# yehonatan145/PatternMatching

Hardware: AMD Instinct MI355X
Metric: GB/s stream scanned + matches/sec, snort.dict, 1/2/4/8 MI355X vs CPU ref (higher is better)
Workload: dtype u8

## Files before the change

patternmatching_amd/csrc/pm_kernels.hip:

```cpp
#include <type_traits>

#include <algorithm>

#include "pm_kernels.h"
#include "pm_streamgen.h"

namespace {

#ifdef RT_PLAIN_STORES
#define RT_OUT_STORE(v, p) (*(p) = (v))
#else
#define RT_OUT_STORE(v, p) __builtin_nontemporal_store((v), (p))
#endif
constexpr int RT_THREADS = 1024;
constexpr int RT_WAVES = RT_THREADS / 64;
constexpr int RT_T2_U16 = 65536;
constexpr int RT_FILTER_WORDS = 4096;
constexpr int RT_F3_WORDS = 256;
constexpr int RT_F2_WORDS = 2048;
constexpr uint32_t RT_QCAP = 64;
constexpr uint32_t RT_ROUND = 40;
constexpr int RT_CHUNK = 1024;
constexpr uint32_t CONT16 = 0x8000u;
constexpr uint32_t CONT32 = 0x80000000u;
// ... 105 lines not shown
        } else {
            const uint32_t ch = wide_child(t.wide[(size_t)R.z * 4 + (c >> 6)], c);
            if (ch == ~0u) return R.y;
            node = ch;
        }
        ++d;
    }
}

__device__ __forceinline__ uint32_t rt_slot1(uint32_t k, uint32_t bits) { return rt_hash(k) >> (32 - bits); }
__device__ __forceinline__ uint32_t rt_slot2(uint32_t k, uint32_t bits) { return (k * 0x85EBCA77u) >> (32 - bits); }

template <bool FOLD = false>
__device__ __forceinline__ uint32_t rt_from_d2(const uint8_t* __restrict__ text, const RtDev& t, uint32_t key24,
                                               uint32_t c3, uint32_t best2, int64_t i, int64_t avail) {
    const uint32_t want = T3H_VALID | key24;
    uint4 e = t.t3h[rt_slot1(key24, t.t3h_bits)];
    if ((e.x & 0x1FFFFFFu) != want) {
        e = t.t3h[rt_slot2(key24, t.t3h_bits)];
        if ((e.x & 0x1FFFFFFu) != want) return best2;
    }
    const uint32_t kind = e.x >> 25;
    if (kind == 0 || avail < 4) return e.y;
    if (kind == 1) {
        const uint32_t nch = e.z >> 24;
        const uint32_t k = c3 == (e.z & 0xFFu) ? 0u : c3 == ((e.z >> 8) & 0xFFu) ? 1u : c3 == ((e.z >> 16) & 0xFFu) ? 2u : 3u;
        if (k >= nch) return e.y;
        if (nch > 1) return rt_deep<FOLD>(text, t, e.w + k, i, avail, 4);
        if (!(e.w & CONT32)) return e.w;
        return rt_deep<FOLD>(text, t, e.w & 0x7FFFFFFFu, i, avail, 4);
    }
    return rt_deep<FOLD>(text, t, e.w & 0x7FFFFFFFu, i, avail, 3);
}

template <bool FOLD = false>
__device__ uint32_t rt_one(const uint8_t* __restrict__ text, const uint16_t* s_t, const RtDev& t, int64_t i,
                           int64_t stream_start) {
    const int64_t avail = i - stream_start + 1;
    const uint32_t c0 = rt_byte<FOLD>(text, i);
    if (avail == 1) return t.t12[65536 + c0];
    const uint32_t c1 = rt_byte<FOLD>(text, i - 1);
    const uint32_t v = s_t[(c0 << 8) | c1];
    if (!(v & CONT16) || avail == 2) return v & 0x7FFFu;
    return rt_from_d2<FOLD>(text, t, rt_byte<FOLD>(text, i - 2) | (c1 << 8) | (c0 << 16),
                            avail >= 4 ? rt_byte<FOLD>(text, i - 3) : 0u, v & 0x7FFFu, i, avail);
}

template <int OUTW>
__device__ __forceinline__ void put_id(void* out, int64_t k, uint32_t v) {
    if (OUTW == 4) reinterpret_cast<uint32_t*>(out)[k] = v;
    if (OUTW == 2) reinterpret_cast<uint16_t*>(out)[k] = (uint16_t)v;
}

template <int I, int N, class F>
__device__ __forceinline__ void unroll_for(F&& f) {
    if constexpr (I < N) {
        f(std::integral_constant<int, I>{});
        unroll_for<I + 1, N>(f);
    }
}

using tu32x2 = __attribute__((ext_vector_type(2))) unsigned int;
using tu32x4 = __attribute__((ext_vector_type(4))) unsigned int;

constexpr int RT_PROBE_G = 4;
constexpr int RT_TAIL_SLOTS = 4;
constexpr uint32_t RT_D4 = 1u << 30;
enum : uint32_t { TS_EMPTY = 0, TS_ENTRY, TS_REC, TS_WIDE };

struct TailSlot {
    uint32_t st;
    uint32_t pos;
    uint32_t av;
    uint32_t node, dd;
    uint32_t c;
    uint32_t tlo, thi;
    int32_t twa;
    const tu32x4* pa;
    const tu32x2* pb;
    tu32x4 A;
    tu32x2 B;
};

template <int OUTW, bool kProbeOnly = false, int SLOTS = RT_TAIL_SLOTS>
__device__ __forceinline__ uint32_t rt_tail(const uint8_t* __restrict__ text, int64_t stream_start, int64_t pos0,
                                        void* __restrict__ out, const RtDev& t, const uint32_t* s_f2,
                                        uint32_t* sp, uint32_t sn, int lane, uint32_t& cnt) {
    const uint8_t* const tb = text + pos0;
    const int64_t ctx64 = pos0 - stream_start;
    const uint32_t ctx = ctx64 > 1024 ? 1024u : (uint32_t)ctx64;
    const tu32x4* const dummy4 = reinterpret_cast<const tu32x4*>(t.filt);
    const tu32x2* const dummy2 = reinterpret_cast<const tu32x2*>(t.filt);
    const tu32x4* const T3 = reinterpret_cast<const tu32x4*>(t.t3h);
    const tu32x4* const RC = reinterpret_cast<const tu32x4*>(t.rec);
    const tu32x4* const WD = reinterpret_cast<const tu32x4*>(t.wide);
    tu32x2* const items = reinterpret_cast<tu32x2*>(sp);

    uint32_t nwalk = 0;
    for (uint32_t base = 0; base < sn; base += 64 * RT_PROBE_G) {
        tu32x2 it[RT_PROBE_G];
        tu32x4 e[RT_PROBE_G];
        bool act[RT_PROBE_G];
        unroll_for<0, RT_PROBE_G>([&](auto g) __attribute__((always_inline)) {
            const uint32_t idx = base + 64 * g + lane;
            it[g] = idx < sn ? items[idx] : tu32x2{0u, 0u};
            act[g] = idx < sn && rt_stage2_hit(rt_stage2_load(s_f2, it[g].x)) != 0u;
        });
        unroll_for<0, RT_PROBE_G>([&](auto g) __attribute__((always_inline)) {
            e[g] = act[g] ? T3[rt_slot1(it[g].x >> 8, t.t3h_bits)] : *dummy4;
        });
        bool need2[RT_PROBE_G];
        bool any2 = false;
        unroll_for<0, RT_PROBE_G>([&](auto g) __attribute__((always_inline)) {
            const uint32_t want = T3H_VALID | (it[g].x >> 8);
            need2[g] = act[g] && (e[g].x & 0x1FFFFFFu) != want && (e[g].x & T3H_VALID);
            any2 |= need2[g];
        });
        if (__ballot(any2)) {
            unroll_for<0, RT_PROBE_G>([&](auto g) __attribute__((always_inline)) {
                if (need2[g]) e[g] = T3[rt_slot2(it[g].x >> 8, t.t3h_bits)];
            });
        }
        unroll_for<0, RT_PROBE_G>([&](auto g) __attribute__((always_inline)) {
            const tu32x4 E = e[g];
            const uint32_t key = it[g].x, pw = it[g].y, off = pw & RT_POSMASK;
            const bool match = act[g] && (E.x & 0x1FFFFFFu) == (T3H_VALID | (key >> 8));
            const uint32_t kind = E.x >> 25, nch = E.z >> 24, c3 = key & 0xFFu;
            const uint32_t j = c3 == (E.z & 0xFFu) ? 0u : c3 == ((E.z >> 8) & 0xFFu) ? 1u
                             : c3 == ((E.z >> 16) & 0xFFu) ? 2u : 3u;
            const bool deep4 = off + ctx >= 3;
            const bool inl = kind == 1 && j < nch && nch == 1 && !(E.w & CONT32);
            const bool walk = match && deep4 && ((kind == 1 && j < nch && !inl) || kind == 2);
            const uint32_t node = (kind == 2 || nch == 1) ? E.w & 0x7FFFFFFFu : E.w + j;
            const uint32_t ans = (deep4 && inl) ? E.w : E.y;
            if (match && !walk) {
                cnt += (uint32_t)(ans != 0u) - (pw >> 31);
                if (OUTW) put_id<OUTW>(out, (int64_t)off, ans);
            }
            const uint64_t m = __ballot(walk);
            if (walk) items[nwalk + wave_prefix(m)] = tu32x2{node, (pw & ~RT_D4) | (kind == 1 ? RT_D4 : 0u)};
            nwalk += (uint32_t)__popcll(m);
        });
    }
    if (!nwalk || kProbeOnly) return nwalk;
    __builtin_amdgcn_s_waitcnt(0);
    __builtin_amdgcn_fence(__ATOMIC_ACQUIRE, "agent");

    TailSlot S[SLOTS];
    unroll_for<0, SLOTS>([&](auto I) __attribute__((always_inline)) {
        TailSlot& z = S[I];
        z.st = TS_EMPTY;
        z.pos = z.av = z.node = z.dd = z.c = z.tlo = z.thi = 0;
        z.twa = 0;
        z.pa = dummy4;
        z.pb = dummy2;
        z.A = tu32x4{0u, 0u, 0u, 0u};
        z.B = tu32x2{0u, 0u};
    });
    uint32_t nxt = 0;
    for (;;) {
        bool busy = false;
        unroll_for<0, SLOTS>([&](auto I) __attribute__((always_inline)) {
            TailSlot& z = S[I];
            const bool need = z.st == TS_EMPTY;
            const uint64_t m = __ballot(need);
            const uint32_t idx = nxt + wave_prefix(m);
            if (need && idx < nwalk) {
                z.st = TS_ENTRY;
                z.c = idx & 1u;
                z.pa = reinterpret_cast<const tu32x4*>(items + (idx & ~1u));
                z.pb = dummy2;
            }
            nxt += (uint32_t)__popcll(m);
            if (nxt > nwalk) nxt = nwalk;
            busy |= z.st != TS_EMPTY;
        });
        if (!__ballot(busy)) break;
        unroll_for<0, SLOTS>([&](auto I) __attribute__((always_inline)) {
            TailSlot& z = S[I];
            z.A = *z.pa;
            z.B = *z.pb;
        });
        unroll_for<0, SLOTS>([&](auto I) __attribute__((always_inline)) {
            TailSlot& z = S[I];
            const uint32_t st = z.st;
            const tu32x4 A = z.A;
            const uint32_t en = z.c ? A.z : A.x, ep = z.c ? A.w : A.y;
            const uint32_t off = z.pos & RT_POSMASK;
            const int32_t rq = (int32_t)off - (int32_t)z.dd;
            const bool reload = rq < z.twa || rq >= z.twa + 8;
            const uint32_t rlo = reload ? z.B.x : z.tlo, rhi = reload ? z.B.y : z.thi;
            const int32_t rta = reload ? (rq & ~7) : z.twa;
            const uint32_t ro = (uint32_t)(rq - rta);
            const uint32_t c = ((ro & 4 ? rhi : rlo) >> (8 * (ro & 3))) & 0xFFu;
            const uint32_t rkind = rec_kind(A), first = A.x & 0xFFFFFFu;
            const uint32_t jr = rec_kid_index(A, c);
            const bool rend = z.dd >= z.av;
            const bool rnext = !rend && rkind == RT_REC_KIDS_K && jr != ((A.x >> 24) & 63u);
            const bool rwide = !rend && rkind == RT_REC_WIDE_K;
            const uint64_t win = ((uint64_t)rhi << 32 | rlo) << (8 * (7 - ro));
            const uint64_t dif = win ^ ((uint64_t)A.w << 32 | A.z);
            const uint32_t meq = dif ? (uint32_t)__builtin_clzll(dif) >> 3 : 8u;
            const uint32_t clen = (A.x >> 24) & 63u;
            const uint32_t cav = z.av > z.dd ? z.av - z.dd : 0u;
            const uint32_t clim = min(min(clen, ro + 1u), cav);
            const uint32_t cm = min(meq, clim);
            const bool cnext = rkind == RT_REC_CHAIN_K && cm >= 1u && (cm == clen || (cm == ro + 1u && cm < cav));
            const uint32_t wnode = wide_child(A, z.c);
            const bool wnext = wnode != ~0u;

            uint32_t nst = TS_EMPTY;
            bool fin = false;
            uint32_t ans = A.w;
            if (st == TS_ENTRY) {
                nst = TS_REC;
                z.node = en;
                z.dd = (ep & RT_D4) ? 4u : 3u;
                z.pos = ep & ~RT_D4;
                const uint32_t o = ep & RT_POSMASK;
                z.av = o + ctx + 1 > 1024u ? 1024u : o + ctx + 1;
                z.twa = INT32_MIN / 2;
            }
            if (st == TS_REC) {
                nst = (rnext || cnext) ? TS_REC : rwide ? TS_WIDE : TS_EMPTY;
                fin = !rnext && !rwide && !cnext;
                ans = A.y;
                z.tlo = rlo;
                z.thi = rhi;
                z.twa = rta;
                z.node = cnext ? first + cm - 1u : first + jr;
                z.dd += rnext ? 1u : cnext ? cm : 0u;
                z.c = c;
            }
            if (st == TS_WIDE) {
                nst = wnext ? TS_REC : TS_EMPTY;
                fin = !wnext;
                z.node = wnode;
                z.dd += 1;
            }
            if (fin) {
                cnt += (uint32_t)(ans != 0u) - (z.pos >> 31);
                if (OUTW) put_id<OUTW>(out, (int64_t)(z.pos & RT_POSMASK), ans);
            }
            z.st = nst;
            const int32_t nq = (int32_t)(z.pos & RT_POSMASK) - (int32_t)z.dd;
            const bool nreload = z.dd < z.av && (nq < z.twa || nq >= z.twa + 8);
            const tu32x4* pa = dummy4;
            const tu32x2* pb = dummy2;
            if (nst == TS_REC) {
                pa = RC + z.node;
                if (nreload) pb = reinterpret_cast<const tu32x2*>(tb + (nq & ~7));
            }
            if (nst == TS_WIDE) pa = WD + (size_t)A.z * 4 + (c >> 6);
            z.pa = pa;
            z.pb = pb;
        });
    }
    return nwalk;
}

template <int V, int OUTW, bool EF = false>
__global__ __launch_bounds__(RT_THREADS) void rt_scan_kernel(const uint8_t* __restrict__ text, int64_t stream_start,
                                                             int64_t pos0, int64_t n, void* __restrict__ out,
                                                             unsigned long long* __restrict__ count, RtDev t) {
    static_assert(V == 0 || V == 2, "product kernel (0) or streaming floor (2)");
    constexpr bool kT8 = V == 0 && OUTW == 0;
    constexpr int kLdsWords = kT8 ? RT_T2_U16 / 4 + RT_F2_WORDS + 2 * RT_WAVES * RT_QCAP
                                  : RT_FILTER_WORDS + RT_T2_U16 / 2 + RT_F2_WORDS + 2 * RT_WAVES * RT_QCAP;
    __shared__ __attribute__((aligned(16))) uint32_t s_lds[kLdsWords];
    uint32_t* const s_f = s_lds;
    const uint8_t* const s_t8 = reinterpret_cast<const uint8_t*>(s_lds);
    const uint16_t* const s_t = kT8 ? t.t12 : reinterpret_cast<uint16_t*>(s_lds + RT_FILTER_WORDS);
    uint32_t* const s_f2 = s_lds + (kT8 ? RT_T2_U16 / 4 : RT_FILTER_WORDS + RT_T2_U16 / 2);
    uint32_t(*const s_qkey)[RT_QCAP] = reinterpret_cast<uint32_t(*)[RT_QCAP]>(s_f2 + RT_F2_WORDS);
    uint32_t(*const s_qpos)[RT_QCAP] = s_qkey + RT_WAVES;
    {
        const uint4* fsrc = reinterpret_cast<const uint4*>(t.filt);
        if (kT8) {
            const uint2* src = reinterpret_cast<const uint2*>(t.t12);
            for (int k = threadIdx.x; k < RT_T2_U16 / 4; k += RT_THREADS) {
                const uint2 v = src[k];
                const uint32_t e[4] = {v.x & 0xFFFFu, v.x >> 16, v.y & 0xFFFFu, v.y >> 16};
                uint32_t w = 0;
#pragma unroll
                for (int q = 0; q < 4; ++q) {
                    const uint32_t nz = (e[q] & 0x7FFFu) != 0u, cand = !nz && (e[q] & CONT16);
                    w |= (nz | cand << 1) << (8 * q);
                }
                s_lds[k] = w;
            }
        } else {
            const uint4* src = reinterpret_cast<const uint4*>(t.t12);
            uint4* dst = reinterpret_cast<uint4*>(s_lds + RT_FILTER_WORDS);
            for (int k = threadIdx.x; k < RT_T2_U16 * 2 / 16; k += RT_THREADS) dst[k] = src[k];
            uint4* fdst = reinterpret_cast<uint4*>(s_f);
            for (int k = threadIdx.x; k < RT_FILTER_WORDS / 4; k += RT_THREADS) fdst[k] = fsrc[k];
        }
        uint4* f2dst = reinterpret_cast<uint4*>(s_f2);
        for (int k = threadIdx.x; k < RT_F2_WORDS / 4; k += RT_THREADS) f2dst[k] = fsrc[RT_FILTER_WORDS / 4 + k];
    }
    __syncthreads();

    constexpr bool kFilter = V == 0;
    constexpr bool kPushS2 = V == 0 && OUTW == 4;
    constexpr bool kRounds = !(V == 0 && OUTW == 0);
    constexpr bool kStage1 = !(V == 0 && OUTW == 0);
    const int lane = threadIdx.x & 63;
    const int wid = __builtin_amdgcn_readfirstlane(threadIdx.x >> 6);
    uint32_t* qkey = s_qkey[wid];
    uint32_t* qpos = s_qpos[wid];
    uint32_t cnt = 0;
    uint32_t scnt = 0;
    const int64_t nchunks = (n + RT_CHUNK - 1) / RT_CHUNK;
    const int64_t c_hi = n / RT_CHUNK;
    const int64_t c_lo = pos0 - stream_start >= 2 ? 0 : 1;
    const int64_t gw = (int64_t)blockIdx.x * RT_WAVES + wid;
    const int64_t nw = (int64_t)gridDim.x * RT_WAVES;
    const int64_t cbeg = c_lo + gw, cend = c_hi, cstep = nw;
    uint32_t* const sp = t.spill + 2 * gw * t.spill_stride;
    uint32_t sn = 0;
    const uint8_t* dummy = reinterpret_cast<const uint8_t*>(t.filt) + 4;
    using u32x2 = __attribute__((ext_vector_type(2))) unsigned int;
    using u32x4 = __attribute__((ext_vector_type(4))) unsigned int;

    struct Round {
        uint32_t n;
        uint32_t keep;
        uint32_t fk, fp;
        u32x2 tw;
        uint32_t skip;
        u32x4 L0;
    };
    uint32_t qh = 0, qn = 0;
    auto issue = [&](Round& r, uint32_t take) __attribute__((always_inline)) {
        __builtin_amdgcn_wave_barrier();
        const bool act = (uint32_t)lane < take;
        const uint32_t sl = (qh + lane) & (RT_QCAP - 1);
        r.fk = act ? qkey[sl] : 0u;
        r.fp = act ? qpos[sl] : 0u;
        const bool deep = r.fp >> 31;
        bool skip = false;
        if (!kPushS2 && take) {
            const bool first = act && !deep && !(r.fp & RT_SLOT2);
            if (first) skip = rt_stage2_hit(rt_stage2_load(s_f2, r.fk)) == 0u;
        }
        r.skip = skip;
        r.keep = (uint32_t)__popcll(__ballot(act && !skip));
        const uint32_t k = r.fk >> 8;
        const uint32_t node = r.fk & 0x7FFFFFu, d = r.fk >> 23;
        const bool wide = deep && (r.fp & RT_SLOT2);
        const int64_t i = pos0 + (int64_t)(r.fp & RT_POSMASK);
        const u32x4* T = reinterpret_cast<const u32x4*>(t.t3h);
        const u32x4* F = reinterpret_cast<const u32x4*>(t.filt);
        const uint32_t slot = (r.fp & RT_SLOT2) ? rt_slot2(k, t.t3h_bits) : rt_slot1(k, t.t3h_bits);
        const u32x4* W = reinterpret_cast<const u32x4*>(t.wide) + (size_t)(r.fk & 0x3FFFu) * 4 + ((r.fk >> 20) & 3u);
        const u32x4* a0 = wide ? W : deep ? reinterpret_cast<const u32x4*>(t.rec) + node : ((act && !skip) ? T + slot : F);
        const uint8_t* a1 = (deep && !wide && (int64_t)d <= i - stream_start) ? text + ((i - d) & ~(int64_t)7) : dummy;
        r.L0 = *a0;
        r.tw = *reinterpret_cast<const u32x2*>(a1);
        r.n = take;
        qh += take;
        qn -= take;
    };
    auto consume = [&](Round& r) __attribute__((always_inline)) {
        u32x4 L0 = r.L0;
        u32x2 tw = r.tw;
        uint32_t fk = r.fk, fp = r.fp;
        asm volatile("" : "+v"(L0), "+v"(tw), "+v"(fk), "+v"(fp)::"memory");
        bool again = false, wstep = false;
        uint32_t nk = 0, np = 0;
        if ((uint32_t)lane < r.n && !r.skip) {
            const int64_t i = pos0 + (int64_t)(fp & RT_POSMASK);
            const int64_t avail = i - stream_start + 1;
            uint32_t v, ph0 = 0xFFFFFFFFu, node = 0, d = 0;
            bool reprobe = false;
            if (!(fp >> 31)) {
                const uint32_t k = fk >> 8, c3 = fk & 0xFFu;
                ph0 = s_t[k >> 8] & 0x7FFFu;
                const uint32_t want = T3H_VALID | k;
                const u32x4 e = L0;
                v = ph0;
                if ((e.x & 0x1FFFFFFu) != want && (e.x & T3H_VALID) && !(fp & RT_SLOT2)) {
                    reprobe = true;
                    again = true;
                } else if ((e.x & 0x1FFFFFFu) == want) {
                    v = e.y;
                    const uint32_t kind = e.x >> 25;
                    if (avail >= 4 && kind == 1) {
                        const uint32_t nch = e.z >> 24;
                        const uint32_t j = c3 == (e.z & 0xFFu) ? 0u : c3 == ((e.z >> 8) & 0xFFu) ? 1u
                                         : c3 == ((e.z >> 16) & 0xFFu) ? 2u : 3u;
                        if (j < nch) {
                            if (nch == 1 && !(e.w & CONT32)) {
                                v = e.w;
                            } else {
                                again = true;
                                node = nch == 1 ? e.w & 0x7FFFFFFFu : e.w + j;
                                d = 4;
                            }
                        }
                    } else if (avail >= 4 && kind == 2) {
                        again = true;
                        node = e.w & 0x7FFFFFFFu;
                        d = 3;
                    }
                }
            } else if (fp & RT_SLOT2) {
                const uint32_t ch = wide_child(L0, (fk >> 14) & 0xFFu);
                d = (fk >> 22) + 1;
                v = L0.w;
                if (ch != ~0u) {
                    node = ch;
                    again = true;
                }
            } else {
                d = fk >> 23;
                const u32x4 R = L0;
                v = R.y;
                if ((int64_t)d < avail) {
                    const uint32_t kind = rec_kind(R);
                    const uint32_t ro = (uint32_t)(i - d) & 7u;
                    const uint32_t tc = (((ro & 4) ? tw.y : tw.x) >> (8 * (ro & 3))) & 0xFFu;
                    if (kind == RT_REC_CHAIN_K) {
                        const uint64_t win = ((uint64_t)tw.y << 32 | tw.x) << (8 * (7 - ro));
                        const uint64_t dif = win ^ ((uint64_t)R.w << 32 | R.z);
                        const uint32_t meq = dif ? (uint32_t)__builtin_clzll(dif) >> 3 : 8u;
                        const uint32_t clen = (R.x >> 24) & 63u;
                        const uint32_t cav = (uint32_t)(avail - d);
                        const uint32_t cm = min(meq, min(min(clen, ro + 1u), cav));
                        if (cm >= 1u && (cm == clen || (cm == ro + 1u && cm < cav))) {
                            node = (R.x & 0xFFFFFFu) + cm - 1u;
                            d += cm;
                            again = true;
                        }
                    } else if (kind == RT_REC_KIDS_K) {
                        const uint32_t j = rec_kid_index(R, tc);
                        if (j != ((R.x >> 24) & 63u)) {
                            node = (R.x & 0xFFFFFFu) + j;
                            ++d;
                            again = true;
                        }
                    } else if (kind == RT_REC_WIDE_K) {
                        wstep = true;
                        again = true;
                        node = R.z | (tc << 14);
                    }
                }
            }
            if (reprobe) {
                nk = fk;
                np = fp | RT_SLOT2;
            } else if (wstep) {
                nk = node | (d << 22);
                np = fp | RT_SLOT2;
            } else if (again) {
                nk = node | (d << 23);
                np = (fp & ~RT_SLOT2) | 0x80000000u;
                if (!(fp >> 31)) cnt -= (uint32_t)(ph0 != 0u);
            } else {
                cnt += (uint32_t)(v != 0u) - ((fp >> 31) ? 0u : (uint32_t)(ph0 != 0u));
                if (OUTW && v != ph0) put_id<OUTW>(out, i - pos0, v);
            }
        }
        __builtin_amdgcn_wave_barrier();
        const uint64_t m = __ballot(again);
        if (again) {
            const uint32_t sl = (qh + qn + wave_prefix(m)) & (RT_QCAP - 1);
            qkey[sl] = nk;
            qpos[sl] = np;
        }
        __builtin_amdgcn_wave_barrier();
        qn += (uint32_t)__popcll(m);
        r.n = 0;
        r.keep = 0;
    };
    auto fetch = [&](uint32_t (&xr)[4], uint32_t& xp, int64_t c) __attribute__((always_inline)) {
        const uint8_t* base = c < cend ? text + pos0 + c * RT_CHUNK : dummy;
#pragma unroll
        for (int s = 0; s < 4; ++s)
            xr[s] = __builtin_nontemporal_load(reinterpret_cast<const uint32_t*>(base + 256 * s + 4 * lane));
        xp = __builtin_nontemporal_load(reinterpret_cast<const uint32_t*>(base - 4));
    };
    auto stand_in_store = [&]() __attribute__((always_inline)) {
        if (OUTW == 4) {
            u32x4* o = reinterpret_cast<u32x4*>(t.scratch);
#pragma unroll
            for (int s = 0; s < 4; ++s) __builtin_nontemporal_store(u32x4{0u, 0u, 0u, 0u}, o + 64 * s + lane);
        }
        if (OUTW == 2) {
            u32x2* o = reinterpret_cast<u32x2*>(t.scratch);
#pragma unroll
            for (int s = 0; s < 4; ++s) __builtin_nontemporal_store(u32x2{0u, 0u}, o + 64 * s + lane);
        }
    };
    Round rr;
    rr.n = 0;
    rr.keep = 0;
    uint32_t xa[4], xb[4], pa, pb;
    int64_t ch = cbeg;
    const uint32_t scap = (uint32_t)t.spill_stride;
    auto resolve = [&]() __attribute__((always_inline)) {
        if (!kFilter) return;
        if (rr.n) consume(rr);
        while (qn) {
            Round rs;
            issue(rs, qn);
            consume(rs);
        }
        if (kRounds && t.spill_total && sn && lane == 0) atomicAdd(t.spill_total, (unsigned long long)sn);
        __builtin_amdgcn_s_waitcnt(0);
        {
            const uint32_t nwalk = rt_tail<OUTW>(text, stream_start, pos0, out, t, s_f2, sp, sn, lane, cnt);
            if (!kRounds && t.spill_total && nwalk && lane == 0)
                atomicAdd(t.spill_total, (unsigned long long)nwalk);
        }
        __builtin_amdgcn_s_waitcnt(0);
        sn = 0;
    };
    auto chunk = [&](uint32_t (&xr)[4], uint32_t& xp, int64_t c) __attribute__((always_inline)) {
        const int64_t pc = pos0 + c * RT_CHUNK;
        u32x2 x[4];
#pragma unroll
        for (int s = 0; s < 4; ++s) {
            const uint32_t fix = s == 0 ? xp : __builtin_amdgcn_update_dpp(0u, xr[s - 1], 0x13C, 0xf, 0xf, false);
            x[s].x = __builtin_amdgcn_update_dpp(fix, xr[s], 0x138, 0xf, 0xf, false);
            x[s].y = xr[s];
        }
        if (EF) fetch(xr, xp, c + 2 * cstep);
#define RT_RAW(j) ((uint32_t)((((uint64_t)x[(j) >> 2].y << 32) | x[(j) >> 2].x) >> (8 * (2 + ((j) & 3)))))
#define RT_KEY(j) (RT_RAW(j) & 0xFFFFFFu)
        uint32_t res[16];
        constexpr int CMS = kT8 ? 1 : 0;
        uint32_t cm = 0;
        if (kT8) {
            uint32_t f = 0;
            constexpr uint32_t kSel0 = 0x0C0C0000u;
#define RT_T8KEY(j) \
    __builtin_amdgcn_perm(x[(j) >> 2].y, x[(j) >> 2].x, kSel0 | (4u + ((j) & 3)) << 8 | (3u + ((j) & 3)))
#pragma unroll
            for (int j = 0; j < 16; ++j) f |= (uint32_t)s_t8[RT_T8KEY(j)] << (2 * j);
#undef RT_T8KEY
            cnt += (uint32_t)__popc(f & 0x55555555u);
            cm = f & 0xAAAAAAAAu;
        } else {
#pragma unroll
        for (int j = 0; j < 16; ++j) res[j] = V == 2 ? RT_KEY(j) & 0xFFFFu : s_t[RT_KEY(j) >> 8];
        if (kFilter && kStage1) {
            uint32_t fw[16];
#pragma unroll
            for (int j = 0; j < 16; ++j) fw[j] = s_f[rt_fhash(RT_RAW(j)) >> 20];
#pragma unroll
            for (int j = 0; j < 16; ++j) cm |= ((res[j] >> 15) & rt_fhit(fw[j], rt_fhash(RT_RAW(j)))) << j;
        } else if (kFilter) {
#pragma unroll
            for (int j = 0; j < 16; ++j) cm |= (res[j] >> 15) << j;
        }
        if (kFilter) {
            if (OUTW == 0) {
                uint32_t zm = 0;
#pragma unroll
                for (int j = 0; j < 16; ++j) zm |= (uint32_t)((res[j] & 0x7FFFu) == 0u) << j;
                cm &= zm;
            }
        }
#pragma unroll
        for (int j = 0; j < 16; ++j) {
            res[j] &= 0x7FFFu;
            scnt += (uint32_t)__popcll(__ballot(res[j] != 0u));
        }
        }
#undef RT_KEY
#undef RT_RAW
        if (kFilter && kRounds) {
            if (rr.n) consume(rr);
            issue(rr, qn >= RT_ROUND ? qn : 0u);
        }
        if (OUTW == 4) {
            u32x4* o = reinterpret_cast<u32x4*>(reinterpret_cast<uint32_t*>(out) + (pc - pos0));
#pragma unroll
            for (int s = 0; s < 4; ++s) {
                u32x4 v = {res[4 * s], res[4 * s + 1], res[4 * s + 2], res[4 * s + 3]};
                RT_OUT_STORE(v, o + 64 * s + lane);
            }
        }
        if (OUTW == 2) {
            u32x2* o = reinterpret_cast<u32x2*>(reinterpret_cast<uint16_t*>(out) + (pc - pos0));
#pragma unroll
            for (int s = 0; s < 4; ++s) {
                u32x2 v = {res[4 * s] | (res[4 * s + 1] << 16), res[4 * s + 2] | (res[4 * s + 3] << 16)};
                RT_OUT_STORE(v, o + 64 * s + lane);
            }
        }
        asm volatile("" ::: "memory");
        if (kPushS2) {
            uint32_t mm = cm, keep = 0;
            while (mm) {
                const uint32_t bit = __builtin_ctz(mm), j = bit >> CMS;
                mm &= mm - 1;
                const uint32_t sg = j >> 2, b = j & 3;
                const u32x2 w01 = (sg & 1) ? x[1] : x[0], w23 = (sg & 1) ? x[3] : x[2];
                const u32x2 w = (sg & 2) ? w23 : w01;
                const uint32_t q32 = (uint32_t)((((uint64_t)w.y << 32) | w.x) >> (8 * (1 + b)));
                keep |= (rt_stage2_hit(rt_stage2_load(s_f2, q32)) != 0u) << bit;
            }
            cm = keep;
        }
        if (kFilter) {
            const uint32_t c = __popc(cm);
            const uint32_t incl = wave_scan_incl(c);
            const uint32_t base = incl - c;
            const uint32_t total = __builtin_amdgcn_readlane(incl, 63);
            uint32_t mm = cm;
            const uint32_t pbase = (uint32_t)(pc - pos0) + 4 * lane;
            if (kRounds && total <= RT_QCAP - qn - rr.keep) {
                uint32_t slot = qh + qn + base;
                while (mm) {
                    const uint32_t j = __builtin_ctz(mm) >> CMS;
                    mm &= mm - 1;
                    const uint32_t sg = j >> 2, b = j & 3;
                    const u32x2 w01 = (sg & 1) ? x[1] : x[0], w23 = (sg & 1) ? x[3] : x[2];
                    const u32x2 w = (sg & 2) ? w23 : w01;
                    const uint32_t sl = slot & (RT_QCAP - 1);
                    qkey[sl] = (uint32_t)((((uint64_t)w.y << 32) | w.x) >> (8 * (1 + b)));
                    qpos[sl] = pbase + 256 * sg + b;
                    ++slot;
                }
                qn += total;
            } else {
                uint32_t room = kRounds ? RT_QCAP - qn - rr.keep : 0u;
                if (__builtin_expect(sn + (total - room) > scap, 0)) {
                    resolve();
                    room = kRounds ? min(RT_QCAP, total) : 0u;
                }
                uint32_t rank = base;
                while (mm) {
                    const uint32_t j = __builtin_ctz(mm) >> CMS;
                    mm &= mm - 1;
                    const uint32_t sg = j >> 2, b = j & 3;
                    const u32x2 w01 = (sg & 1) ? x[1] : x[0], w23 = (sg & 1) ? x[3] : x[2];
                    const u32x2 w = (sg & 2) ? w23 : w01;
                    const uint32_t q32 = (uint32_t)((((uint64_t)w.y << 32) | w.x) >> (8 * (1 + b)));
                    const uint32_t p = pbase + 256 * sg + b;
                    if (rank < room) {
                        const uint32_t sl = (qh + qn + rank) & (RT_QCAP - 1);
                        qkey[sl] = q32;
                        qpos[sl] = p;
                    } else {
                        const uint32_t ph = OUTW == 0 ? 0u : (uint32_t)((s_t[q32 >> 16] & 0x7FFFu) != 0u);
                        reinterpret_cast<u32x2*>(sp)[sn + rank - room] = u32x2{q32, p | (ph << 31)};
                    }
                    ++rank;
                }
                sn = __builtin_amdgcn_readfirstlane(sn + total - room);
                qn = __builtin_amdgcn_readfirstlane(qn + room);
            }
        }
        if (!EF) fetch(xr, xp, c + 2 * cstep);
    };
    Round r0;
    if (EF) fetch(xa, pa, ch);
    if (kFilter && kRounds) issue(r0, 0);
    stand_in_store();
    if (!EF) fetch(xa, pa, ch);
    if (EF) fetch(xb, pb, ch + cstep);
    if (kFilter && kRounds) issue(rr, 0);
    stand_in_store();
    if (!EF) fetch(xb, pb, ch + cstep);
    for (;;) {
        if (ch >= cend) break;
        chunk(xa, pa, ch);
        if (ch + cstep >= cend) break;
        chunk(xb, pb, ch + cstep);
        ch += 2 * cstep;
    }
    resolve();
    if (blockIdx.x == gridDim.x - 1) {
#pragma unroll 1
        for (int e = 0; e < 2; ++e) {
            int64_t c = -1;
            if (e == 0 && c_lo == 1) c = 0;
            if (e == 1 && c_hi < nchunks && !(c_lo == 1 && c_hi == 0)) c = c_hi;
            const int64_t p = pos0 + c * RT_CHUNK + threadIdx.x;
            if (c >= 0 && p < pos0 + n) {
                const uint32_t v = rt_one(text, s_t, t, p, stream_start);
                if (OUTW) put_id<OUTW>(out, p - pos0, v);
                cnt += v != 0u;
            }
        }
    }
    if (count) {
        for (int o = 32; o > 0; o >>= 1) cnt += __shfl_down(cnt, o);
        cnt += scnt;
        if (lane == 0 && cnt) atomicAdd(count, (unsigned long long)cnt);
    }
}

constexpr int RT_SMALL_THREADS = 256;
template <int OUTW>
__global__ __launch_bounds__(RT_SMALL_THREADS) void rt_small_kernel(const uint8_t* __restrict__ text,
                                                                    int64_t stream_start, int64_t pos0, int64_t n,
                                                                    void* __restrict__ out,
                                                                    unsigned long long* __restrict__ count, RtDev t) {
    const int64_t k = (int64_t)blockIdx.x * RT_SMALL_THREADS + threadIdx.x;
    uint32_t v = 0, deep = 0;
    if (k < n) {
        const int64_t i = pos0 + k;
        v = rt_one(text, t.t12, t, i, stream_start);
        if (t.spill_total && i - stream_start >= 3 && (t.t12[(uint32_t)text[i] << 8 | text[i - 1]] & CONT16)) {
            const uint32_t q = (uint32_t)text[i - 3] | (uint32_t)text[i - 2] << 8 | (uint32_t)text[i - 1] << 16 |
                               (uint32_t)text[i] << 24;
            const uint32_t f = rt_fhash(q >> 8);
            if (rt_fhit(t.filt[f >> 20], f)) deep = rt_stage2_hit(rt_stage2_load(t.filt + RT_FILTER_WORDS, q));
        }
        if (OUTW) put_id<OUTW>(out, k, v);
    }
    const uint64_t nz = __ballot(v != 0u), dp = __ballot(deep != 0u);
    if ((threadIdx.x & 63) == 0) {
        if (count && nz) atomicAdd(count, (unsigned long long)__popcll(nz));
        if (t.spill_total && dp) atomicAdd(t.spill_total, (unsigned long long)__popcll(dp));
    }
}

constexpr int RT_SERVE_WIN = 16384;
constexpr int RT_SERVE_POLLERS = 4;
#ifndef PM_SERVE_TRACE
#define PM_SERVE_TRACE 0
#endif
__device__ __forceinline__ uint64_t rfl64(uint64_t x) {
    const uint32_t lo = __builtin_amdgcn_readfirstlane((uint32_t)x);
    const uint32_t hi = __builtin_amdgcn_readfirstlane((uint32_t)(x >> 32));
    return (uint64_t)hi << 32 | lo;
}
__device__ __forceinline__ uint64_t lane64(uint64_t x, int l) {
    const uint32_t lo = __builtin_amdgcn_readlane((uint32_t)x, l);
    const uint32_t hi = __builtin_amdgcn_readlane((uint32_t)(x >> 32), l);
    return (uint64_t)hi << 32 | lo;
}
template <class T>
__device__ __forceinline__ T sys_load(const T* p) {
    return __hip_atomic_load(p, __ATOMIC_RELAXED, __HIP_MEMORY_SCOPE_SYSTEM);
}
template <class T>
__device__ __forceinline__ void sys_store(T* p, T v) {
    __hip_atomic_store(p, v, __ATOMIC_RELAXED, __HIP_MEMORY_SCOPE_SYSTEM);
}
template <class T>
__device__ __forceinline__ T dev_load(const T* p) {
    return __hip_atomic_load(p, __ATOMIC_RELAXED, __HIP_MEMORY_SCOPE_AGENT);
}
template <class T>
__device__ __forceinline__ void dev_store(T* p, T v) {
    __hip_atomic_store(p, v, __ATOMIC_RELAXED, __HIP_MEMORY_SCOPE_AGENT);
}
__global__ __launch_bounds__(RT_SERVE_THREADS) void rt_serve_kernel(PmServeReq* req, uint64_t* fwd, uint32_t* done,
                                                                    uint64_t seen, uint64_t gen, int64_t idle_ticks,
                                                                    RtDev t) {
    __shared__ __attribute__((aligned(16))) uint8_t win[RT_SERVE_WIN];
    __shared__ uint64_t s_w[8];
    __shared__ uint32_t s_state;
    const uint64_t* const rq = reinterpret_cast<const uint64_t*>(req);
    const int tid = threadIdx.x;
    const int wid = __builtin_amdgcn_readfirstlane(tid >> 6);
    const int64_t G = gridDim.x, wg = blockIdx.x;
    if (tid == 0) s_state = 0;
    __syncthreads();
    for (;;) {
        if (wg == 0 ? wid < RT_SERVE_POLLERS : wid == 0) {
            for (int q = 0; q < wid; ++q) __builtin_amdgcn_s_sleep(24);
            const uint64_t t0 = __builtin_amdgcn_s_memrealtime();
            uint64_t w = 0;
            uint32_t found = 0, quit = 0;
            const uint64_t* const src = wg == 0 ? rq : fwd;
            for (;;) {
                w = wg == 0 ? sys_load(src + (tid & 7)) : dev_load(src + (tid & 7));
                const uint64_t s2 = lane64(w, 7);
                if (s2 > seen && s2 == lane64(w, 0)) {
                    found = 1;
                    break;
                }
                if (lane64(w, 1) == gen || __builtin_amdgcn_s_memrealtime() - t0 > (uint64_t)idle_ticks) {
                    quit = 1;
                    break;
                }
                if (wg == 0 && __builtin_amdgcn_readfirstlane(
                                   __hip_atomic_load(&s_state, __ATOMIC_RELAXED, __HIP_MEMORY_SCOPE_WORKGROUP)))
                    break;
                __builtin_amdgcn_s_sleep(1);
            }
#if PM_SERVE_TRACE
            if ((tid & 63) == 0 && wg < 2 && found)
                sys_store(reinterpret_cast<uint64_t*>(done + G + 16) + 8 * wg, __builtin_amdgcn_s_memrealtime());
#endif
            if (found) {
                const int lane = tid & 63;
                uint32_t old = 1;
                if (lane == 0) old = __hip_atomic_exchange(&s_state, 1u, __ATOMIC_RELAXED, __HIP_MEMORY_SCOPE_WORKGROUP);
                if (__builtin_amdgcn_readfirstlane(old) != 1) {
                    if (lane < 8 && lane != 1) s_w[lane] = w;
                    if (wg == 0) {
                        if (lane >= 2 && lane < 7) dev_store(fwd + lane, w);
                        __builtin_amdgcn_s_waitcnt(0);
                        if (lane == 0 || lane == 7) dev_store(fwd + lane, w);
                    }
                }
            } else if (quit && (tid & 63) == 0) {
                uint32_t zero = 0;
                __hip_atomic_compare_exchange_strong(&s_state, &zero, 2u, __ATOMIC_RELAXED, __ATOMIC_RELAXED,
                                                     __HIP_MEMORY_SCOPE_WORKGROUP);
            }
        }
        __syncthreads();
        if (__builtin_amdgcn_readfirstlane(s_state) == 2) {
            if (wg == 0 && tid == 1) dev_store(fwd + 1, gen);
            return;
        }
        __syncthreads();
        if (tid == 0) s_state = 0;
        const uint64_t v = rfl64(s_w[0]);
        seen = v;
        const uint8_t* const text = reinterpret_cast<const uint8_t*>(rfl64(s_w[2]));
        void* const out = reinterpret_cast<void*>(rfl64(s_w[3]));
        const int64_t ss = (int64_t)rfl64(s_w[4]), pos0 = (int64_t)rfl64(s_w[5]);
        const uint64_t nw = rfl64(s_w[6]);
        const int64_t n = (int64_t)(nw & ((1ull << 56) - 1));
        const bool w4 = (nw >> 56) == 4;
        const int64_t per = ((n + G - 1) / G + 63) & ~(int64_t)63;
        const int64_t a = wg * per < n ? wg * per : n, b = a + per < n ? a + per : n;
        if (a < b) {
            const int64_t back = (int64_t)t.back + 4;
            const int64_t lo = (pos0 + a - back > ss ? pos0 + a - back : ss) & ~(int64_t)7;
            const int64_t hi = (pos0 + b + 7) & ~(int64_t)7;
            if (hi - lo <= RT_SERVE_WIN) {
                for (int64_t k = 8 * tid; k < hi - lo; k += 8 * RT_SERVE_THREADS)
                    *reinterpret_cast<uint64_t*>(win + k) = sys_load(reinterpret_cast<const uint64_t*>(text + lo + k));
                __syncthreads();
#if PM_SERVE_TRACE
                if (tid == 0 && wg < 2)
                    sys_store(reinterpret_cast<uint64_t*>(done + G + 16) + 8 * wg + 1, __builtin_amdgcn_s_memrealtime());
#endif
                for (int64_t k = a + tid; k < b; k += RT_SERVE_THREADS) {
                    const uint32_t r = rt_one(win, t.t12, t, pos0 + k - lo, ss - lo);
                    if (w4) reinterpret_cast<uint32_t*>(out)[k] = r;
                    else reinterpret_cast<uint16_t*>(out)[k] = (uint16_t)r;
                }
            } else {
                for (int64_t k = a + tid; k < b; k += RT_SERVE_THREADS) {
                    const uint32_t r = rt_one(text, t.t12, t, pos0 + k, ss);
                    if (w4) reinterpret_cast<uint32_t*>(out)[k] = r;
                    else reinterpret_cast<uint16_t*>(out)[k] = (uint16_t)r;
                }
            }
        }
#if PM_SERVE_TRACE
        if (tid == 0 && wg < 2)
            sys_store(reinterpret_cast<uint64_t*>(done + G + 16) + 8 * wg + 2, __builtin_amdgcn_s_memrealtime());
#endif
        __builtin_amdgcn_s_waitcnt(0);
        __syncthreads();
#if PM_SERVE_TRACE
        if (tid == 0 && wg < 2)
            sys_store(reinterpret_cast<uint64_t*>(done + G + 16) + 8 * wg + 3, __builtin_amdgcn_s_memrealtime());
#endif
        if (tid == 0) __hip_atomic_store(done + wg, (uint32_t)v, __ATOMIC_RELEASE, __HIP_MEMORY_SCOPE_SYSTEM);
#if PM_SERVE_TRACE
        if (tid == 0 && wg < 2)
            sys_store(reinterpret_cast<uint64_t*>(done + G + 16) + 8 * wg + 4, __builtin_amdgcn_s_memrealtime());
#endif
    }
}

constexpr int RT_BATCH_TILE = RT_THREADS;

__device__ __forceinline__ int64_t batch_seek(const int64_t* __restrict__ offs, int64_t lo, int64_t cnt, int64_t key) {
    int64_t hi = lo, step = 1;
    while (hi < cnt && (int64_t)rfl64((uint64_t)offs[hi]) < key) {
        lo = hi + 1;
        hi += step;
        step <<= 1;
    }
    if (hi > cnt) hi = cnt;
    while (lo < hi) {
        const int64_t mid = lo + ((hi - lo) >> 1);
        if ((int64_t)rfl64((uint64_t)offs[mid]) < key) lo = mid + 1;
        else hi = mid;
    }
    return lo;
}

template <int OUTW, bool SMALL>
__global__ __launch_bounds__(RT_THREADS) void rt_batch_kernel(const uint8_t* __restrict__ text,
                                                              const int64_t* __restrict__ offs, int64_t nseg,
                                                              int64_t n, void* __restrict__ out,
                                                              unsigned long long* __restrict__ count, RtDev t) {
    constexpr int kT12Words = SMALL ? 0 : RT_T2_U16 / 2;
    __shared__ __attribute__((aligned(16))) uint32_t s_lds[kT12Words + RT_BATCH_TILE / 32];
    uint32_t* const s_mask = s_lds + kT12Words;
    const uint16_t* s_t = t.t12;
    const int tid = threadIdx.x;
    if (!SMALL) {
        const uint4* src = reinterpret_cast<const uint4*>(t.t12);
        uint4* dst = reinterpret_cast<uint4*>(s_lds);
        for (int k = tid; k < RT_T2_U16 * 2 / 16; k += RT_THREADS) dst[k] = src[k];
        __syncthreads();
        s_t = reinterpret_cast<const uint16_t*>(s_lds);
    }
    const int64_t ntiles = (n + RT_BATCH_TILE - 1) / RT_BATCH_TILE;
    const int64_t T0 = ntiles * (int64_t)blockIdx.x / (int64_t)gridDim.x;
    const int64_t T1 = ntiles * ((int64_t)blockIdx.x + 1) / (int64_t)gridDim.x;
    const int64_t noffs = nseg + 1;
    int64_t a = batch_seek(offs, 0, noffs, T0 * RT_BATCH_TILE + 1);
// ... 3032 lines not shown
```

Baseline: 917.4.

## Compact stage-1 candidates into queue before lane-parallel stage-2 filtering

Instead of each lane serially probing the stage-2 filter for its own candidate bits, candidates are first pushed into the per-wave LDS queue, then each lane checks one queued entry against stage 2 and survivors are re-compacted with a ballot prefix. This is meant to remove divergent per-lane loops in the stage-2 check. Several A/B macros are added for experiments, and the old path remains as a fallback when the queue would overflow. The added wave barriers, LDS round trips and the fallback's use of `bit` without `>> CMS` in the new loop risk extra cost or inconsistency.

```diff
diff --git a/patternmatching_amd/csrc/pm_kernels.hip b/patternmatching_amd/csrc/pm_kernels.hip
--- a/patternmatching_amd/csrc/pm_kernels.hip
+++ b/patternmatching_amd/csrc/pm_kernels.hip
@@ -431,7 +431,11 @@
     __syncthreads();
 
     constexpr bool kFilter = V == 0;
+#ifdef RT_AB_U16_PUSH
+    constexpr bool kPushS2 = V == 0 && OUTW != 0;
+#else
     constexpr bool kPushS2 = V == 0 && OUTW == 4;
+#endif
     constexpr bool kRounds = !(V == 0 && OUTW == 0);
     constexpr bool kStage1 = !(V == 0 && OUTW == 0);
     const int lane = threadIdx.x & 63;
@@ -721,7 +725,60 @@
             }
         }
         asm volatile("" ::: "memory");
+#ifdef RT_AB_DROP_PASSERS
         if (kPushS2) {
+            asm volatile("" ::"v"(cm));
+            cm = 0;
+        }
+#endif
+        bool pushed = false;
+#ifndef RT_AB_LANE_S2
+        if (kPushS2) {
+            const uint32_t c = __popc(cm);
+            const uint32_t incl = wave_scan_incl(c);
+            const uint32_t total = __builtin_amdgcn_readlane(incl, 63);
+            if (total <= RT_QCAP - qn) {
+                uint32_t mm = cm, slot = qh + qn + incl - c;
+                const uint32_t pbase = (uint32_t)(pc - pos0) + 4 * lane;
+                while (mm) {
+                    const uint32_t j = __builtin_ctz(mm);
+                    mm &= mm - 1;
+                    const uint32_t sg = j >> 2, b = j & 3;
+                    const u32x2 w01 = (sg & 1) ? x[1] : x[0], w23 = (sg & 1) ? x[3] : x[2];
+                    const u32x2 w = (sg & 2) ? w23 : w01;
+                    const uint32_t sl = slot & (RT_QCAP - 1);
+                    qkey[sl] = (uint32_t)((((uint64_t)w.y << 32) | w.x) >> (8 * (1 + b)));
+                    qpos[sl] = pbase + 256 * sg + b;
+                    ++slot;
+                }
+                __builtin_amdgcn_wave_barrier();
+                const uint32_t sl = (qh + qn + lane) & (RT_QCAP - 1);
+                const uint32_t k = qkey[sl], p = qpos[sl];
+#ifdef RT_AB_KEEP_ALL
+                const bool kp = (uint32_t)lane < total;
+#else
+                const uint32_t hit = rt_stage2_hit(rt_stage2_load(s_f2, k));
+                const bool kp = ((uint32_t)lane < total) & (hit != 0u);
+#endif
+                const uint64_t m = __ballot(kp);
+                const uint32_t nk = (uint32_t)__popcll(m);
+                if (nk <= RT_QCAP - qn - rr.keep) {
+                    if (kp) {
+                        const uint32_t ks = (qh + qn + wave_prefix(m)) & (RT_QCAP - 1);
+                        qkey[ks] = k;
+                        qpos[ks] = p;
+                    }
+                    qn += nk;
+                    pushed = true;
+                }
+                __builtin_amdgcn_wave_barrier();
+            }
+#ifdef RT_AB_COUNT_OVERFLOW
+            if (!pushed && lane == 0 && count) atomicAdd(count, 1ull << 40);
+#endif
+        }
+#endif
+        if (kPushS2 && !pushed) {
             uint32_t mm = cm, keep = 0;
             while (mm) {
                 const uint32_t bit = __builtin_ctz(mm), j = bit >> CMS;
@@ -732,9 +789,11 @@
                 const uint32_t q32 = (uint32_t)((((uint64_t)w.y << 32) | w.x) >> (8 * (1 + b)));
                 keep |= (rt_stage2_hit(rt_stage2_load(s_f2, q32)) != 0u) << bit;
             }
+#ifndef RT_AB_KEEP_ALL
             cm = keep;
-        }
-        if (kFilter) {
+#endif
+        }
+        if (kFilter && !pushed) {
             const uint32_t c = __popc(cm);
             const uint32_t incl = wave_scan_incl(c);
             const uint32_t base = incl - c;
```

After: 923.8, median of 6. Within noise of the previous version (+0.7%).
